# haliphinx/TCE-RVOS

Measured on AMD Instinct MI355X. Metric: clips/s (T=5, 360×640, Swin-T) at 1/2/4/8 MI355X; mask IoU vs ref, higher is better.
Workload: dtype f32 (3xf16-split MFMA, f32 accumulate); 1 GPU; swin_t_p4w7 T=5 360x640 + 32-token text, B=1 clip per forward, flags --with_box_refine --binary --f_token 8 --qtrans (BASELINE config 2); clips_in_flight_per_gpu=1, clips_per_forward=1, same_clip_in_group=False, ranks_per_gpu=1, parallelism=clip-sharded x1

## Files before the change

include/tce_rvos_debug.h:

```cpp
#ifndef TCE_RVOS_DEBUG_H
#define TCE_RVOS_DEBUG_H
#include <stdint.h>
#ifdef __cplusplus
extern "C" {
#endif
int tce_gemm_force_tile(int32_t tile);
int tce_debug_set_stamp_buffer(long long* dev_buf);
int tce_debug_set_epilogue(int32_t lds_staged);
int tce_debug_ffn_set_stamp_buffer(long long* dev_buf);
int tce_debug_ffn_set_half(int32_t mode);
int tce_debug_msda_set_lds(int32_t on);
int tce_debug_window_attn_set_mfma(int32_t on);
int tce_debug_mha_set_split(int32_t on);
int tce_debug_msda_set_fewq(int32_t on);
int tce_debug_conv3x3_set_waves(int32_t waves);
int tce_debug_conv3x3_set_pieces(int32_t pieces);
#ifdef __cplusplus
}
#endif
#endif
```

tce-rvos_amd/_lib.py:

```python
import ctypes as C
import os

HERE = os.path.dirname(os.path.abspath(__file__))
LIB_PATH = os.environ.get("TCE_LIB") or os.path.join(HERE, "lib", "libtce_rvos.so")

c_f = C.c_void_p
i32, i64, f32 = C.c_int32, C.c_int64, C.c_float


class GemmArgs(C.Structure):
    _fields_ = [("A", c_f), ("A2", c_f), ("W", c_f), ("bias", c_f), ("res", c_f), ("C", c_f),
                ("M", i32), ("N", i32), ("K", i32),
                ("lda", i32), ("lda2", i32), ("ldw", i32), ("ldc", i32), ("ldres", i32),
                ("act", i32), ("res_mode", i32), ("batch", i32),
                ("sA", i64), ("sA2", i64), ("sW", i64), ("sBias", i64), ("sC", i64), ("sRes", i64),
                ("conv", i32), ("T", i32), ("H", i32), ("Wd", i32), ("Cin", i32), ("Ho", i32), ("Wo", i32),
                ("kh", i32), ("kw", i32), ("stride", i32), ("pad", i32)]


class RowLinArgs(C.Structure):
    _fields_ = [("x", c_f), ("a2", c_f), ("packed", c_f), ("bias", c_f), ("res", c_f), ("out", c_f),
                ("g_in", c_f), ("be_in", c_f), ("g_out", c_f), ("be_out", c_f),
                ("ldx", i64), ("lda2", i64), ("ldres", i64), ("ldo", i64),
                ("sX", i64), ("sA2", i64), ("sRes", i64), ("sOut", i64),
# ... 92 lines not shown
    "tce_ffn_packed_bytes": (i64, [i32, i32]),
    "tce_ffn_pack_f32": (i32, [c_f, c_f, c_f, c_f, i32, i32, c_f]),
    "tce_ffn_fused_f32": (i32, [c_f, i64, c_f, c_f, c_f, c_f, f32, c_f, c_f, f32, c_f, i64, i32, i32, i32, i32, c_f]),
    "tce_ffn_split_ws_floats": (i64, [i32, i32, i32, i32]),
    "tce_ffn_split_counters": (i32, [i32, i32, i32, i32]),
    "tce_ffn_set_wg_cap": (i32, [i32]),
    "tce_ffn_capped_grid": (i32, [i32, i32, i32, C.POINTER(i32)]),
    "tce_ffn_fused_split_f32": (i32, [c_f, i64, c_f, c_f, c_f, c_f, f32, c_f, c_f, f32, c_f, i64, i32, i32, i32, i32, c_f, i64, c_f, i32, c_f]),
    "tce_xattn_prepare_f32": (i32, [c_f, c_f, c_f, c_f, c_f, c_f, c_f, i32, i32, i32, c_f]),
    "tce_ffn_pack_batched_f32": (i32, [c_f, c_f, c_f, c_f, i32, i32, i32, c_f]),
    "tce_xattn_fused_f32": (i32, [C.POINTER(XattnArgs), c_f]),
    "tce_xattn_ffn_fused_f32": (i32, [C.POINTER(XattnArgs), C.POINTER(XattnFfnArgs), c_f]),
    "tce_ffn_pack_chain_f32": (i32, [c_f, c_f, c_f, c_f, i32, i32, c_f]),
    "tce_xattn_pack_f32": (i32, [c_f, c_f, c_f, c_f, c_f, i32, i32, i32, c_f]),
    "tce_xattn_prepare_lens_f32": (i32, [c_f, c_f, c_f, c_f, c_f, c_f, c_f, i32, i32, i32, c_f, c_f]),
    "tce_xattn_pack_lens_f32": (i32, [c_f, c_f, c_f, c_f, c_f, i32, i32, i32, c_f, c_f]),
    "tce_rowlin_packed_bytes": (i64, [i32, i32]),
    "tce_rowlin_pack_f32": (i32, [c_f, i64, c_f, i32, i32, c_f]),
    "tce_rowlin_f32": (i32, [C.POINTER(RowLinArgs), c_f]),
    "tce_conv3x3_packed_bytes": (i64, [i32, i32]),
    "tce_conv3x3_pack_f32": (i32, [c_f, c_f, i32, i32, c_f]),
    "tce_conv3x3_f32": (i32, [c_f, i64, c_f, c_f, c_f, i64, i32, i32, i32, i32, i32, c_f]),
    "tce_conv3x3_split_ws_floats": (i64, [i32, i32, i32]),
    "tce_conv3x3_split_pieces": (i32, [i32, i32, i32]),
    "tce_conv3x3_split_kstep": (i32, [i32, i32]),
    "tce_conv3x3_split_f32": (i32, [c_f, i64, c_f, c_f, c_f, i64, i32, i32, i32, i32, i32, c_f, i64, c_f]),
    "tce_fewrow_linear_f32": (i32, [C.POINTER(FewRowArgs), c_f]),
    "tce_thin_linear_splits": (i32, [i32, i32, i32]),
    "tce_thin_partials_f32": (i32, [c_f, i64, i32, c_f, i32, c_f, i64, c_f, i32, i32, i32, c_f]),
    "tce_splitk_reduce_f32": (i32, [c_f, i32, i32, i32, c_f, i32, c_f, i32, i32, c_f, i32, c_f, c_f, f32, c_f]),
    "tce_mha_small64_splits_f32": (i32, [c_f, i32, c_f, c_f, i32, i32, f32, c_f]),
    "tce_swin_attn_packed_bytes": (i64, [i32]),
    "tce_swin_attn_pack_f32": (i32, [c_f, c_f, c_f, i32, c_f]),
    "tce_swin_attn_fused_f32": (i32, [c_f, i64, c_f, c_f, c_f, c_f, c_f, c_f, f32, c_f, i64, i32, i32, i32, i32, i32, c_f]),
    "tce_graph_begin": (i32, [c_f]),
    "tce_graph_end": (i32, [c_f, C.POINTER(C.c_void_p)]),
    "tce_graph_launch": (i32, [C.c_void_p, c_f]),
    "tce_graph_destroy": (i32, [C.c_void_p]),
    "tce_graph_group": (i32, [C.POINTER(C.c_void_p), i32, C.POINTER(C.c_void_p)]),
}

DEBUG_SIGNATURES = {
    "tce_gemm_force_tile": (i32, [i32]),
    "tce_debug_set_stamp_buffer": (i32, [c_f]),
    "tce_debug_set_epilogue": (i32, [i32]),
    "tce_debug_ffn_set_stamp_buffer": (i32, [c_f]),
    "tce_debug_ffn_set_half": (i32, [i32]),
    "tce_debug_msda_set_lds": (i32, [i32]),
    "tce_debug_window_attn_set_mfma": (i32, [i32]),
    "tce_debug_mha_set_split": (i32, [i32]),
    "tce_debug_msda_set_fewq": (i32, [i32]),
    "tce_debug_conv3x3_set_waves": (i32, [i32]),
    "tce_debug_conv3x3_set_pieces": (i32, [i32]),
}

VIDEO_SIGNATURES = {
    "tce_label_objects_u8": (i32, [C.POINTER(LabelObj), i32, c_f, c_f, i32, i32, i32, i32, i32, i32, i32, f32, f32, c_f]),
}

EVAL_SIGNATURES = {
    "tce_a2d_masks_u8": (i32, [c_f, c_f, i32, i32, i32, i32, i32, i32, i32, f32, c_f]),
    "tce_rle_ws_bytes": (i64, [i32, i32, i32]),
    "tce_rle_counts_u32": (i32, [c_f, c_f, c_f, c_f, i32, i32, i32, c_f]),
}

_LIB = None


class TceError(RuntimeError):
    pass


def lib():
    global _LIB
    if _LIB is None:
        if not os.path.exists(LIB_PATH):
            raise TceError(f"{LIB_PATH} not found: build the HIP extension first "
                           f"(python -c 'import __graft_entry__ as g; g.build()'); there is no fallback path")
        hwq = os.environ.get("GPU_MAX_HW_QUEUES")
        if hwq not in (None, "", "4"):
            import warnings
            warnings.warn(f"tce_rvos_amd: GPU_MAX_HW_QUEUES={hwq} is set; the HIP runtime's default (4) is the only value this "
                          f"launch program runs well with (1-3 crash the runtime, 5-16 double the clip time)", RuntimeWarning)
        l = C.CDLL(LIB_PATH)
        for name, (res, args) in list(SIGNATURES.items()) + list(DEBUG_SIGNATURES.items()) + list(VIDEO_SIGNATURES.items()) + \
                list(EVAL_SIGNATURES.items()):
            fn = getattr(l, name)
            fn.restype = res
            fn.argtypes = args
        _LIB = l
    return _LIB


def lib_raw():
    l = lib()
    return l.__dict__.get("_real", l)


def check(status, what=""):
    if status != 0:
        msg = lib().tce_last_error().decode(errors="replace")
        raise TceError(f"{what} failed ({status}): {msg}")
```

tce-rvos_amd/csrc/chain.hip:

```cpp
#include "common.h"
#include "gemm_epilogue.h"
#include "frag.h"
#include "../../include/tce_rvos.h"
#include "../../include/tce_rvos_debug.h"

namespace {

#ifndef FFN_ABL
#define FFN_ABL 0
#endif
static __device__ long long* g_ffn_stamps = nullptr;


template <int K, bool HAS_A2 = true>
__device__ __forceinline__ void load_x_frags(const float* __restrict__ x, const long long ldx,
                                             const float* __restrict__ a2, const long long lda2, const int a2_rows,
                                             const int m0, const int M, float* __restrict__ wt, const int lane,
                                             const float* __restrict__ g_in, const float* __restrict__ be_in,
                                             const float eps, h16x8 (&xh)[K / 16], h16x8 (&xl)[K / 16],
                                             const int single = 0) {
  constexpr int NP = K / 32;
  const int cr = lane >> 3, cp = (lane & 7) * 4;
  const int r = lane & 31, hf = lane >> 5;
  f32x4 v[NP][4];
// ... 1074 lines not shown
    } else {
      const int idx = (p_hi - 1 - 2 * KS) >> 1, t = idx >> 1, s2 = idx & 1, chunk = it - 1;
#pragma unroll
      for (int e = 0; e < 8; ++e) {
        const int col = 32 * chunk + 16 * s2 + 8 * (e >> 2) + 4 * hf + (e & 3);
        const int h = col / G, j = col - h * G;
        val[e] = (chunk >= 0 && chunk < NC && j < Lb) ? dot32(wo + (long long)(32 * t + r) * C + h * HD, v + j * C + h * HD) : 0.f;
      }
    }
    const HL f = split8(val, single);
    oh = __builtin_bit_cast(u32x4, f.hi);
    ol = __builtin_bit_cast(u32x4, f.lo);
  }
  stage_out[p_hi * 64 + lane] = oh;
  if (p_lo < P) stage_out[p_lo * 64 + lane] = ol;
}

constexpr int CONV_PAD_STAGES = 6;

struct ConvArgs {
  const float* x;
  const unsigned char* wpk;
  const float* bias;
  float* out;
  long long ldx, ldo;
  int H, W, M;
  int* range_flag;
  int single;
  int m_off;
  int nb, pieces;
  float* ws;
};

constexpr int CONV_ITERS = 12;
__host__ __device__ constexpr int conv3x3_piece_iter(const int pieces, const int s) { return s * CONV_ITERS / pieces; }

#ifndef CONV_ABL
#define CONV_ABL 0
#endif

template <int BYTE_OFF>
__device__ __forceinline__ void gload16(f32x4& dst, const float* ptr) {
  asm volatile("global_load_dwordx4 %0, %1, off offset:%2" : "=v"(dst) : "v"(ptr), "n"(BYTE_OFF) : "memory");
}

template <int I, int N, typename F>
__device__ __forceinline__ void static_for(F&& f) {
  if constexpr (I < N) {
    f(std::integral_constant<int, I>{});
    static_for<I + 1, N>(f);
  }
}

template <int CIN, bool SINGLE, int WAVES = 4, bool SPLIT = false>
__global__ void __launch_bounds__(64 * WAVES, WAVES / 4) conv3x3_kernel(const ConvArgs p) {
  constexpr int NTL = 8;
  constexpr int PW = 16 / WAVES;
  constexpr int STAGE = 2 * NTL * PIECE;
  constexpr int R = 4;
  constexpr int XS = WAVES == 4 ? 6 : 4, LX = XS + 1;
  constexpr int NW = WAVES == 4 ? CONV_PAD_STAGES - 2 : 3, LW = NW + 2;
  constexpr int INFLIGHT = (2 + PW) * (LW - 3);
  static_assert(LW <= CONV_PAD_STAGES, "the packed stream's zero padding covers the weight lead");
  constexpr int BODY = 12;
  constexpr int ITERS = 3 * (CIN / 64);
  constexpr int KS = BODY * ITERS;
  static_assert(CIN % 64 == 0, "channel chunks come in groups of four");
  static_assert(BODY % R == 0 && BODY % XS == 0 && BODY % NW == 0 && LX >= LW, "ring positions are compile-time");
  static_assert(WAVES * WT_BYTES <= R * STAGE, "the epilogue's staging tiles alias the ring");
  static_assert(!SPLIT || (ITERS == CONV_ITERS && WAVES == 4 && !SINGLE), "split pieces: CIN = 256, 128-pixel workgroups, split fp16");
  __shared__ __attribute__((aligned(16))) unsigned char smem[R * STAGE];

  const int tid = threadIdx.x, lane = tid & 63;
  const int wave = __builtin_amdgcn_readfirstlane(tid >> 6);
  const int hf = lane >> 5;
  const int blk = SPLIT ? (int)blockIdx.x % p.nb : (int)blockIdx.x;
  const int piece = SPLIT ? (int)blockIdx.x / p.nb : 0;
  const int i0 = SPLIT ? conv3x3_piece_iter(p.pieces, piece) : 0;
  const int i1 = SPLIT ? conv3x3_piece_iter(p.pieces, piece + 1) : ITERS;
  const int m0 = p.m_off + blk * (32 * WAVES) + wave * 32;

  const int m = m0 + (lane & 31);
  const int px = m % p.W, py = (m / p.W) % p.H;
  const float* const zeros = reinterpret_cast<const float*>(p.wpk + (long long)(KS + CONV_PAD_STAGES) * STAGE) + 8 * hf;
  const float* const xme = p.x + (long long)min(m, p.M - 1) * p.ldx + 8 * hf;
  auto iter_ptrs = [&](const int it, const float* (&q)[3]) {
    const int dy = it / (CIN / 64) - 1, cq = it % (CIN / 64);
    const bool row_ok = it < i1 && m < p.M && (unsigned)(py + dy) < (unsigned)p.H;
#pragma unroll
    for (int d = 0; d < 3; ++d) {
      const bool ok = row_ok && (unsigned)(px + d - 1) < (unsigned)p.W;
      q[d] = (ok ? xme + (long long)(dy * p.W + d - 1) * p.ldx : zeros) + 64 * cq;
    }
  };

  const float* wp = reinterpret_cast<const float*>(p.wpk + ((long long)i0 * BODY * STAGE) + (long long)(PW * wave) * PIECE + lane * 16);
  unsigned char* const wdst = smem + (PW * wave) * PIECE + lane * 16;
  f32x4 wr[NW][PW];
  auto wload = [&](f32x4 (&dst)[PW]) {
    if (!(CONV_ABL & 8)) {
      gload16<0>(dst[0], wp);
      gload16<PIECE>(dst[1], wp);
      if constexpr (PW == 4) {
        gload16<2 * PIECE>(dst[2], wp);
        gload16<3 * PIECE>(dst[3], wp);
      }
    }
    wp += STAGE / 4;
  };
  auto wstore = [&](const f32x4 (&src)[PW], const int stage) {
#pragma unroll
    for (int q = 0; q < PW; ++q) *reinterpret_cast<f32x4*>(wdst + stage * STAGE + q * PIECE) = src[q];
  };

  f32x4 xr[XS][2];
  const float* cur[3];
  const float* nxt[3];
  iter_ptrs(i0, cur);
  iter_ptrs(i0 + 1, nxt);
  auto xload = [&](auto jjc, f32x4 (&dst)[2]) {
    constexpr int JJ = decltype(jjc)::value;
    constexpr int J = JJ % BODY;
    const float* const src = JJ < BODY ? cur[J % 3] : nxt[J % 3];
    if (CONV_ABL & 16) return;
    gload16<64 * (J / 3)>(dst[0], src);
    gload16<64 * (J / 3) + 16>(dst[1], src);
  };
  auto wait_loads = [&](auto nc, f32x4 (&xs)[2], f32x4 (&ws)[PW]) {
    constexpr int N = (CONV_ABL & 24) ? 0 : decltype(nc)::value;
    if constexpr (PW == 4) {
      asm volatile("s_waitcnt vmcnt(%6)"
                   : "+v"(xs[0]), "+v"(xs[1]), "+v"(ws[0]), "+v"(ws[1]), "+v"(ws[2]), "+v"(ws[3])
                   : "n"(N)
                   : "memory");
    } else {
      asm volatile("s_waitcnt vmcnt(%4)" : "+v"(xs[0]), "+v"(xs[1]), "+v"(ws[0]), "+v"(ws[1]) : "n"(N) : "memory");
    }
  };
  using nfl = std::integral_constant<int, INFLIGHT>;

  f32x16 acc[NTL];
#pragma unroll
  for (int t = 0; t < NTL; ++t)
#pragma unroll
    for (int i = 0; i < 16; ++i) acc[t][i] = 0.f;
  h16x8 bh, bl;
  static_for<0, LX>([&](auto mc) {
    constexpr int m = decltype(mc)::value - LX;
    if constexpr (m + 2 >= 0) {
      wait_loads(nfl{}, xr[(m + 2) % XS], wr[(m + 2) % NW]);
      wstore(wr[(m + 2) % NW], (m + 2) % R);
      if constexpr (m + 2 == 0) {
        const float f[8] = {xr[0][0][0], xr[0][0][1], xr[0][0][2], xr[0][0][3], xr[0][1][0], xr[0][1][1], xr[0][1][2], xr[0][1][3]};
        const HL b = split8(f, SINGLE ? 1 : 0);
        bh = b.hi;
        bl = b.lo;
        asm volatile("" : "+v"(bh), "+v"(bl));
      }
    }
    if constexpr (m + LX >= 0) xload(std::integral_constant<int, m + LX>{}, xr[(m + LX) % XS]);
    if constexpr (m + LW >= 0) wload(wr[(m + LW) % NW]);
  });
  __syncthreads();
  h16x8 fh[4], fl[4];
  {
    const unsigned char* const st = smem + lane * 16;
    fh[0] = *reinterpret_cast<const h16x8*>(st);
    fl[0] = *reinterpret_cast<const h16x8*>(st + PIECE);
    fh[1] = *reinterpret_cast<const h16x8*>(st + 2 * PIECE);
    fl[1] = *reinterpret_cast<const h16x8*>(st + 3 * PIECE);
  }

  for (int it = i0; it < i1; ++it) {
    static_for<0, BODY>([&](auto jc) {
      constexpr int j = decltype(jc)::value;
      constexpr int nslot = (j + 1) % XS;
      const unsigned char* const st = smem + (j % R) * STAGE + lane * 16;
      unsigned nh[4], nl[4];
      auto tile = [&](auto tc) {
        constexpr int t = decltype(tc)::value;
#if CONV_ABL & 4
        const h16x8 k0 = fh[t % 4], k1 = fl[t % 4], k2 = bh, k3 = bl;
        asm volatile("" : : "v"(k0), "v"(k1), "v"(k2), "v"(k3));
#else
        if constexpr (!SINGLE) {
          acc[t] = __builtin_amdgcn_mfma_f32_32x32x16_f16(fh[t % 4], bl, acc[t], 0, 0, 0);
          acc[t] = __builtin_amdgcn_mfma_f32_32x32x16_f16(fl[t % 4], bh, acc[t], 0, 0, 0);
        }
        acc[t] = __builtin_amdgcn_mfma_f32_32x32x16_f16(fh[t % 4], bh, acc[t], 0, 0, 0);
#endif
      };
      static_for<0, 6>([&](auto tc) {
        constexpr int t = decltype(tc)::value;
        fh[(t + 2) % 4] = *reinterpret_cast<const h16x8*>(st + (2 * t + 4) * PIECE);
        fl[(t + 2) % 4] = *reinterpret_cast<const h16x8*>(st + (2 * t + 5) * PIECE);
        __builtin_amdgcn_sched_barrier(0);
        tile(tc);
        if constexpr (t < 4) {
          const float a = xr[nslot][t >> 1][2 * (t & 1)], b = xr[nslot][t >> 1][2 * (t & 1) + 1];
          if constexpr (SINGLE) {
            nh[t] = __builtin_bit_cast(unsigned, fp16x2_t{(__fp16)a, (__fp16)b});
            nl[t] = 0u;
          } else {
            const fp16x2_t h = __builtin_amdgcn_cvt_pkrtz(a, b);
            nh[t] = __builtin_bit_cast(unsigned, h);
            nl[t] = __builtin_bit_cast(unsigned, __builtin_amdgcn_cvt_pkrtz(a - (float)h[0], b - (float)h[1]));
          }
          asm volatile("" : "+v"(nh[t]), "+v"(nl[t]));
        }
        __builtin_amdgcn_sched_barrier(0);
      });
      wait_loads(nfl{}, xr[(j + 2) % XS], wr[(j + 2) % NW]);
      wstore(wr[(j + 2) % NW], (j + 2) % R);
      if (!(CONV_ABL & 2)) __syncthreads();
      xload(std::integral_constant<int, j + LX>{}, xr[(j + LX) % XS]);
      wload(wr[(j + LW) % NW]);
      {
        const unsigned char* const sn = smem + ((j + 1) % R) * STAGE + lane * 16;
        fh[0] = *reinterpret_cast<const h16x8*>(sn);
        fl[0] = *reinterpret_cast<const h16x8*>(sn + PIECE);
        fh[1] = *reinterpret_cast<const h16x8*>(sn + 2 * PIECE);
        fl[1] = *reinterpret_cast<const h16x8*>(sn + 3 * PIECE);
      }
      __builtin_amdgcn_sched_barrier(0);
      tile(std::integral_constant<int, 6>{});
      tile(std::integral_constant<int, 7>{});
      __builtin_amdgcn_sched_barrier(0);
      bh = __builtin_bit_cast(h16x8, u32x4{nh[0], nh[1], nh[2], nh[3]});
      bl = __builtin_bit_cast(h16x8, u32x4{nl[0], nl[1], nl[2], nl[3]});
    });
#pragma unroll
    for (int d = 0; d < 3; ++d) cur[d] = nxt[d];
    iter_ptrs(it + 2, nxt);
  }
  asm volatile("s_waitcnt vmcnt(0)" ::: "memory");
  __syncthreads();

  float* const wt = reinterpret_cast<float*>(smem + wave * WT_BYTES);
  tce_amax_t amax = 0;
  if constexpr (SPLIT) {
    float* const part = p.ws + (long long)piece * (p.M - p.m_off) * 256;
#pragma unroll
    for (int t = 0; t < NTL; ++t) tile_store(acc[t], part, 256, m0 - p.m_off, p.M - p.m_off, 32 * t, wt, lane, amax);
    return;
  }
  const ResTile none = {};
#pragma unroll
  for (int t = 0; t < NTL; ++t) {
    tile_bias_res<0>(acc[t], tile_bias_load(p.bias, 32 * t, lane), none, wt, lane);
    tile_store(acc[t], p.out, p.ldo, m0, p.M, 32 * t, wt, lane, amax);
  }
  tce_range_report(p.range_flag, amax);
}

__global__ void __launch_bounds__(256) conv3x3_reduce_kernel(const float* __restrict__ ws, const int pieces, const int rows,
                                                             const float* __restrict__ bias, float* __restrict__ out,
                                                             const long long ldo, const int m_off, int* range_flag) {
  const long long n4 = (long long)rows * 64, stride = (long long)gridDim.x * 256;
  tce_amax_t amax = 0;
  for (long long i = (long long)blockIdx.x * 256 + threadIdx.x; i < n4; i += stride) {
    const f32x4* src = reinterpret_cast<const f32x4*>(ws) + i;
    f32x4 v = src[0];
    for (int s = 1; s < pieces; ++s) v += src[(long long)s * n4];
    const int c4 = (int)(i & 63);
    if (bias) v += reinterpret_cast<const f32x4*>(bias)[c4];
    amax = tce_amax4(amax, v);
    *reinterpret_cast<f32x4*>(out + (m_off + (i >> 6)) * ldo + 4 * c4) = v;
  }
  tce_range_report(range_flag, amax);
}

__global__ void __launch_bounds__(256) conv3x3_pack_kernel(const float* __restrict__ w, unsigned char* __restrict__ out,
                                                           const int CIN, const long long units, const int single) {
  const long long u = (long long)blockIdx.x * 256 + threadIdx.x;
  if (u >= units) return;
  const int lane = (int)(u & 63);
  const long long pg = u >> 6;
  const int piece = (int)(pg & 15);
  const long long s = pg >> 4;
  const int r = lane & 31, hf = lane >> 5, t = piece >> 1;
  u32x4 o = {0u, 0u, 0u, 0u};
  if (s < 9 * CIN / 16) {
    const int it = (int)(s / 12), j = (int)(s % 12);
    const int dy = it / (CIN / 64), cc = 4 * (it % (CIN / 64)) + j / 3, dx = j % 3;
    float v[8];
#pragma unroll
// ... 433 lines not shown
                     (unsigned char*)packed, Cin, units, tce_gemm_single_pass());
  TCE_CHECK_LAUNCH("tce_conv3x3_pack_f32");
  return TCE_OK;
}

static int g_conv3_waves = 0;
extern "C" int tce_debug_conv3x3_set_waves(int32_t waves) {
  TCE_CHECK_ARG(waves == 0 || waves == 4 || waves == 8, "tce_debug_conv3x3_set_waves: 0 (automatic), 4 or 8");
  g_conv3_waves = waves;
  return TCE_OK;
}

struct Conv3Plan {
  int wide = 4;
  int full8 = 0;
  int m_narrow = 0;
  int nb = 0;
  int pieces = 1;
  long long ws_floats = 0;
};
inline Conv3Plan conv3x3_plan(const int M, const int cus, const int single, const int force_waves, const int split, const int force_pieces) {
  Conv3Plan pl;
  const int r4 = tce_cdiv(tce_cdiv(M, 128), cus), r8 = tce_cdiv(tce_cdiv(M, 256), cus);
  const int full8 = tce_cdiv(M, 256) / cus;
  const int rem_px = M - full8 * 256 * cus;
  const int mixed4 = 7 * full8 + 4 * tce_cdiv(tce_cdiv(rem_px, 128), cus);
  if (!force_waves && !single && full8 >= 1 && rem_px > 0 && mixed4 < 4 * r4 && mixed4 < 7 * r8) {
    pl.full8 = full8 * cus;
    pl.m_narrow = full8 * 256 * cus;
  } else {
    pl.wide = force_waves ? force_waves : (4 * r4 > 7 * r8 ? 8 : 4);
    if (single) pl.wide = 4;
    if (pl.wide == 8) return pl;
  }
  pl.nb = tce_cdiv(M - pl.m_narrow, 128);
  if (!split || single || pl.nb >= cus) return pl;
  const double OVH = 0.5, LAUNCH = 0.3, RED_BPI = 8.0 * (3u << 20);
  const long long px = M - pl.m_narrow;
  auto cost = [&](int p) {
    const double walk = (double)tce_cdiv((long long)pl.nb * p, cus) * (tce_cdiv(CONV_ITERS, p) + OVH);
    return p == 1 ? walk : walk + LAUNCH + (double)(p + 1) * px * 1024.0 / RED_BPI;
  };
  int best = 1;
  for (int p = 2; p <= 6; ++p)
    if ((long long)pl.nb * p <= 2ll * cus && cost(p) < cost(best)) best = p;
  if (force_pieces > 0) best = force_pieces;
  if (best > 1) {
    pl.pieces = best;
    pl.ws_floats = (long long)best * px * 256;
  }
  return pl;
}

static int g_conv3_pieces = 0;
extern "C" int tce_debug_conv3x3_set_pieces(int32_t pieces) {
  TCE_CHECK_ARG(pieces >= 0 && pieces <= CONV_ITERS, "tce_debug_conv3x3_set_pieces: 0 (automatic) .. 12");
  g_conv3_pieces = pieces;
  return TCE_OK;
}

static int conv3_force_waves() {
  static const int env_force = []() { const char* e = getenv("TCE_CONV3_WAVES"); return e ? atoi(e) : 0; }();
  return g_conv3_waves ? g_conv3_waves : env_force;
}

static Conv3Plan conv3x3_plan_for(const int M, const bool split) {
  return conv3x3_plan(M, tce_cu_count(), tce_gemm_single_pass(), conv3_force_waves(), split, g_conv3_pieces);
}

extern "C" int64_t tce_conv3x3_split_ws_floats(int32_t M, int32_t Cin, int32_t N) {
  return conv3x3_shape_ok(Cin, N) && M > 0 ? conv3x3_plan_for(M, true).ws_floats : 0;
}
extern "C" int32_t tce_conv3x3_split_pieces(int32_t M, int32_t Cin, int32_t N) {
  return conv3x3_shape_ok(Cin, N) && M > 0 ? conv3x3_plan_for(M, true).pieces : 0;
}
extern "C" int32_t tce_conv3x3_split_kstep(int32_t pieces, int32_t s) {
  return pieces >= 1 && pieces <= CONV_ITERS && s >= 0 && s <= pieces ? 12 * conv3x3_piece_iter(pieces, s) : -1;
}

static int conv3x3_launch(const float* x, int64_t ldx, const void* packed, const float* bias, float* out, int64_t ldo, int32_t T,
                          int32_t H, int32_t W, int32_t Cin, int32_t N, float* ws, int64_t ws_floats, const bool split, tceStream stream,
                          const char* name) {
  TCE_CHECK_ARG(conv3x3_shape_ok(Cin, N), "%s: unsupported shape Cin=%d N=%d (256 -> 256)", name, Cin, N);
  TCE_CHECK_ARG(x && packed && out && T > 0 && H > 0 && W > 0 && (long long)T * H * W < (1ll << 31),
                "%s: null pointer or bad sizes", name);
  TCE_CHECK_ARG(ldx >= Cin && ldx % 4 == 0 && ldo >= N && ldo % 4 == 0, "%s: bad row pitch", name);
  TCE_CHECK_ARG(tce_aligned16(x) && tce_aligned16(out) && tce_aligned16(packed) && (!bias || tce_aligned16(bias)),
                "%s: pointers must be 16-byte aligned", name);
  ConvArgs a;
  a.x = x; a.wpk = (const unsigned char*)packed; a.bias = bias; a.out = out;
  a.ldx = ldx; a.ldo = ldo; a.H = H; a.W = W; a.M = T * H * W;
  a.range_flag = tce_range_flag(); a.single = tce_gemm_single_pass();
  a.m_off = 0; a.nb = 0; a.pieces = 1; a.ws = nullptr;
  hipStream_t s = (hipStream_t)stream;
  const Conv3Plan pl = conv3x3_plan_for(a.M, split);
  if (pl.pieces > 1)
    TCE_CHECK_ARG(ws && tce_aligned16(ws) && ws_floats >= pl.ws_floats,
                  "%s: workspace of %lld floats needed (tce_conv3x3_split_ws_floats), %lld given", name, pl.ws_floats, (long long)ws_floats);
  if (pl.full8) hipLaunchKernelGGL((conv3x3_kernel<256, false, 8>), dim3(pl.full8), dim3(512), 0, s, a);
  a.m_off = pl.m_narrow;
  if (pl.wide == 8) hipLaunchKernelGGL((conv3x3_kernel<256, false, 8>), dim3(tce_cdiv(a.M, 256)), dim3(512), 0, s, a);
  else if (a.single) hipLaunchKernelGGL((conv3x3_kernel<256, true>), dim3(pl.nb), dim3(256), 0, s, a);
  else if (pl.pieces == 1) hipLaunchKernelGGL((conv3x3_kernel<256, false>), dim3(pl.nb), dim3(256), 0, s, a);
  else {
    a.nb = pl.nb; a.pieces = pl.pieces; a.ws = ws;
    hipLaunchKernelGGL((conv3x3_kernel<256, false, 4, true>), dim3(pl.nb * pl.pieces), dim3(256), 0, s, a);
    const int rows = a.M - a.m_off;
    hipLaunchKernelGGL(conv3x3_reduce_kernel, dim3(std::min(tce_cdiv((long long)rows * 64, 256), 8 * tce_cu_count())), dim3(256), 0, s,
                       (const float*)ws, pl.pieces, rows, bias, out, ldo, a.m_off, a.range_flag);
  }
  TCE_CHECK_LAUNCH(name);
  return TCE_OK;
}

extern "C" int tce_conv3x3_f32(const float* x, int64_t ldx, const void* packed, const float* bias, float* out, int64_t ldo,
                               int32_t T, int32_t H, int32_t W, int32_t Cin, int32_t N, tceStream stream) {
  return conv3x3_launch(x, ldx, packed, bias, out, ldo, T, H, W, Cin, N, nullptr, 0, false, stream, "tce_conv3x3_f32");
}

extern "C" int tce_conv3x3_split_f32(const float* x, int64_t ldx, const void* packed, const float* bias, float* out, int64_t ldo,
                                     int32_t T, int32_t H, int32_t W, int32_t Cin, int32_t N, float* ws, int64_t ws_floats,
                                     tceStream stream) {
  return conv3x3_launch(x, ldx, packed, bias, out, ldo, T, H, W, Cin, N, ws, ws_floats, true, stream, "tce_conv3x3_split_f32");
}

bool tce_patch_embed_mfma(const float* frames, const float* w, const float* b, const float* gamma, const float* beta,
                          float* out, int H, int W, int C, float eps, long long ntok, int Hp, int Wp, hipStream_t s) {
  if ((C != 96 && C != 128 && C != 192) || ntok >= (1ll << 31) || !tce_aligned16(frames) || !tce_aligned16(out) ||
      !tce_aligned16(w) || !tce_aligned16(b) || !tce_aligned16(gamma) || !tce_aligned16(beta))
    return false;
  const dim3 grid(tce_cdiv(ntok, 128)), block(256);
  int* const rf = tce_range_flag();
  const int single = tce_gemm_single_pass();
  if (C == 96) hipLaunchKernelGGL((patch_embed_mfma_kernel<3>), grid, block, 0, s, frames, w, b, gamma, beta, out, H, W, eps, (int)ntok, Hp, Wp, rf, single);
  else if (C == 128) hipLaunchKernelGGL((patch_embed_mfma_kernel<4>), grid, block, 0, s, frames, w, b, gamma, beta, out, H, W, eps, (int)ntok, Hp, Wp, rf, single);
  else hipLaunchKernelGGL((patch_embed_mfma_kernel<6>), grid, block, 0, s, frames, w, b, gamma, beta, out, H, W, eps, (int)ntok, Hp, Wp, rf, single);
  return true;
}
#endif
```

tce-rvos_amd/ops.py:

```python
import ctypes as C

import os
import threading

import torch

from ._lib import GemmArgs, check, lib

ACT_NONE, ACT_RELU, ACT_GELU, ACT_RELU_AFTER_RES = 0, 1, 2, 3
RES_NONE, RES_ADD, RES_MUL = 0, 1, 2


class Arena:

    ALIGN = 256
    FLAGS = 1 << 14

    def __init__(self, device, nbytes):
        self.device = torch.device(device)
        self.buf = torch.empty(int(nbytes), dtype=torch.uint8, device=self.device)
        self.off = 0
        self.peak = 0
        self.flags = torch.zeros(self.FLAGS, dtype=torch.int32, device=self.device)
        self.flag_off = 0
# ... 1043 lines not shown
    if nbytes < 0:
        raise ValueError(f"rowlin_pack: unsupported shape N={N} K={K}")
    out = torch.empty(nbytes, dtype=torch.uint8, device=w.device)
    check(lib().tce_rowlin_pack_f32(w.data_ptr(), ldw, out.data_ptr(), N, K, _stream()), "tce_rowlin_pack_f32")
    return out


def rowlin_register(w, table=None):
    if w.dim() != 2 or w.stride(1) != 1 or w.shape[1] not in ROWLIN_K or w.shape[0] % 32 or not w.is_cuda:
        return None
    r = _ROUTES if table is None else table
    key = (w.data_ptr(), w.shape[0], w.shape[1], w.stride(0), get_gemm_mode())
    if key not in r.rowlin:
        r.rowlin[key] = rowlin_pack(w)
        r.keep.append(w)
    return r.rowlin[key]


def rowlin(x, pk, out, M, N, K, ldx, ldo, bias=None, a2=None, lda2=0, a2_rows=0, act=ACT_NONE, res=None, ldres=0,
           res_mode=RES_NONE, ln_in=None, ln_out=None, eps_in=1e-5, eps_out=1e-5, batch=1, sX=0, sA2=0, sRes=0, sOut=0):
    from ._lib import RowLinArgs
    q = RowLinArgs()
    q.x, q.packed, q.out = x.data_ptr(), pk.data_ptr(), out.data_ptr()
    q.M, q.N, q.K, q.batch = M, N, K, batch
    q.ldx, q.ldo = ldx, ldo
    if a2 is not None:
        q.a2, q.lda2, q.a2_rows = a2.data_ptr(), lda2, a2_rows
    if bias is not None:
        q.bias = bias.data_ptr()
    if res_mode != RES_NONE:
        q.res, q.ldres = res.data_ptr(), ldres
    if ln_in is not None:
        q.g_in, q.be_in = ln_in[0].data_ptr(), ln_in[1].data_ptr()
    if ln_out is not None:
        q.g_out, q.be_out = ln_out[0].data_ptr(), ln_out[1].data_ptr()
    q.act, q.res_mode, q.eps_in, q.eps_out = act, res_mode, eps_in, eps_out
    q.sX, q.sA2, q.sRes, q.sOut = sX, sA2, sRes, sOut

    def go():
        check(lib().tce_rowlin_f32(C.byref(q), _stream()), "tce_rowlin_f32")
    if GEMM_PROFILE is None:
        go()
        return out
    e0, e1 = torch.cuda.Event(enable_timing=True), torch.cuda.Event(enable_timing=True)
    e0.record()
    go()
    e1.record()
    GEMM_PROFILE.append((f"rowlin_kernel<{K}", False, 2.0 * M * N * K * batch, e0, e1))
    return out


CONV3_MIN_PIXELS = int(os.environ.get("TCE_CONV3_MIN_PIXELS", 12000))
CONV3_SPLIT = os.environ.get("TCE_CONV3_SPLIT", "1") != "0"


def conv3x3_split_ws_floats(M, Cin=256, N=256):
    return int(lib().tce_conv3x3_split_ws_floats(M, Cin, N)) if CONV3_SPLIT else 0


def conv3x3_pack(w_cl, Cin):
    _chk(w_cl, "w")
    N = w_cl.shape[0]
    nbytes = lib().tce_conv3x3_packed_bytes(Cin, N)
    if nbytes < 0 or w_cl.shape[1] != 9 * Cin or not w_cl.is_contiguous():
        raise ValueError(f"conv3x3_pack: unsupported shape N={N} Cin={Cin}")
    out = torch.empty(nbytes, dtype=torch.uint8, device=w_cl.device)
    check(lib().tce_conv3x3_pack_f32(w_cl.data_ptr(), out.data_ptr(), Cin, N, _stream()), "tce_conv3x3_pack_f32")
    return out


def conv3x3_register(w_cl, Cin, table=None):
    if lib().tce_conv3x3_packed_bytes(Cin, w_cl.shape[0]) < 0 or w_cl.shape[1] != 9 * Cin:
        return None
    r = _ROUTES if table is None else table
    key = (w_cl.data_ptr(), w_cl.shape[0], w_cl.shape[1], get_gemm_mode())
    if key not in r.conv3:
        r.conv3[key] = conv3x3_pack(w_cl, Cin)
        r.keep.append(w_cl)
    return r.conv3[key]


def conv3x3(x, pk, T, H, W, Cin, N, bias=None, out=None, alloc=None):
    _chk(x, "x")
    M = T * H * W
    if out is None:
        out = alloc(M, N) if alloc else torch.empty(M, N, dtype=torch.float32, device=x.device)

    nws = conv3x3_split_ws_floats(M, Cin, N) if alloc else 0
    ws = alloc(nws) if nws else None

    def go():
        bp = bias.data_ptr() if bias is not None else None
        if ws is not None:
            check(lib().tce_conv3x3_split_f32(x.data_ptr(), x.stride(0), pk.data_ptr(), bp, out.data_ptr(), out.stride(0), T, H, W,
                                              Cin, N, ws.data_ptr(), nws, _stream()), "tce_conv3x3_split_f32")
        else:
            check(lib().tce_conv3x3_f32(x.data_ptr(), x.stride(0), pk.data_ptr(), bp, out.data_ptr(), out.stride(0), T, H, W, Cin,
                                        N, _stream()), "tce_conv3x3_f32")
    if GEMM_PROFILE is None:
        go()
        return out
    e0, e1 = torch.cuda.Event(enable_timing=True), torch.cuda.Event(enable_timing=True)
    e0.record()
    go()
    e1.record()
    GEMM_PROFILE.append((f"conv3x3_kernel<{Cin}", True, 2.0 * M * N * 9 * Cin, e0, e1))
    return out


XATTN_MIN_ROWS = int(os.environ.get("TCE_XATTN_MIN_ROWS", 4000))
XATTN_PACK_FUSED = os.environ.get("TCE_XATTN_PACK_FUSED", "1") != "0"


def xattn_static(wq, bq, scale=32 ** -0.5):
    return (torch.cat([wq.t(), bq[None]], 0) * scale).contiguous()


def xattn_pack(k, v, wqT_ext, wo, L, alloc, group=32, batch=1, lens=None):
    _chk(k, "k")
    _chk(v, "v")
    Hd = 8 * group
    if XATTN_PACK_FUSED:
        pk = alloc(batch, lib().tce_ffn_packed_bytes(256, Hd), dtype=torch.uint8)
        if lens is not None:
            check(lib().tce_xattn_pack_lens_f32(k.data_ptr(), v.data_ptr(), wqT_ext.data_ptr(), wo.data_ptr(), pk.data_ptr(), L, group,
                                                batch, lens.data_ptr(), _stream()), "tce_xattn_pack_lens_f32")
            return pk
        check(lib().tce_xattn_pack_f32(k.data_ptr(), v.data_ptr(), wqT_ext.data_ptr(), wo.data_ptr(), pk.data_ptr(), L, group, batch,
                                       _stream()), "tce_xattn_pack_f32")
        return pk
    W1, b1, W2 = alloc(batch, Hd, 256), alloc(batch, Hd), alloc(batch, 256, Hd)
    if lens is not None:
        check(lib().tce_xattn_prepare_lens_f32(k.data_ptr(), v.data_ptr(), wqT_ext.data_ptr(), wo.data_ptr(), W1.data_ptr(),
                                               b1.data_ptr(), W2.data_ptr(), L, group, batch, lens.data_ptr(), _stream()),
              "tce_xattn_prepare_lens_f32")
    else:
# ... 91 lines not shown
```

Measured before the change: 177.9 clips/s.

## Reuse centre-tap activations across 3x3 conv horizontal taps via DPP lane shifts

The 3x3 conv kernel now loads only the centre column of activations plus a single halo pixel at each end of the 32-pixel wave row, instead of three separate global loads per dy/channel chunk. The left and right taps come from DPP row shifts of the already split fp16 hi/lo values, with explicit zeroing at image borders. This cuts global activation traffic and VMEM requests roughly threefold. The cost is a new load/wait schedule built from constexpr in-flight counts, more registers, and extra DPP/select work. A runtime flag and env var can switch back to the old path.

```diff
diff --git a/include/tce_rvos_debug.h b/include/tce_rvos_debug.h
--- a/include/tce_rvos_debug.h
+++ b/include/tce_rvos_debug.h
@@ -15,6 +15,7 @@
 int tce_debug_msda_set_fewq(int32_t on);
 int tce_debug_conv3x3_set_waves(int32_t waves);
 int tce_debug_conv3x3_set_pieces(int32_t pieces);
+int tce_debug_conv3x3_set_reuse(int32_t reuse);
 #ifdef __cplusplus
 }
 #endif
diff --git a/tce-rvos_amd/_lib.py b/tce-rvos_amd/_lib.py
--- a/tce-rvos_amd/_lib.py
+++ b/tce-rvos_amd/_lib.py
@@ -168,6 +168,7 @@
     "tce_debug_msda_set_fewq": (i32, [i32]),
     "tce_debug_conv3x3_set_waves": (i32, [i32]),
     "tce_debug_conv3x3_set_pieces": (i32, [i32]),
+    "tce_debug_conv3x3_set_reuse": (i32, [i32]),
 }
 
 VIDEO_SIGNATURES = {
diff --git a/tce-rvos_amd/csrc/chain.hip b/tce-rvos_amd/csrc/chain.hip
--- a/tce-rvos_amd/csrc/chain.hip
+++ b/tce-rvos_amd/csrc/chain.hip
@@ -1150,7 +1150,26 @@
   }
 }
 
-template <int CIN, bool SINGLE, int WAVES = 4, bool SPLIT = false>
+template <int LW, int PW, bool PAIR>
+struct ConvReuse {
+  static constexpr int NC = PAIR ? 3 : 2;
+  static constexpr int centre(int c) { return 3 * (PAIR ? (c & ~1) : c) - LW - 1; }
+  static constexpr int halo(int c) { return 3 * c - LW; }
+  static constexpr int cslot(int c) { return PAIR ? ((c & 1) ? 1 + ((c >> 1) & 1) : 0) : (c & 1); }
+  static constexpr int loads(int k) {
+    int n = PW;
+    for (int c = -8; c < 16; ++c) n += 2 * (centre(c) == k) + 2 * (halo(c) == k);
+    return n;
+  }
+  static constexpr int inflight(int j) {
+    int n = 0;
+    for (int k = j + 3 - LW; k <= j - 1; ++k) n += loads(k);
+    return n;
+  }
+  static_assert(centre(-1) < -(LW + 1) && halo(-1) < -(LW + 1), "no request of an earlier iteration falls into the prologue");
+};
+
+template <int CIN, bool SINGLE, int WAVES = 4, bool SPLIT = false, bool REUSE = true>
 __global__ void __launch_bounds__(64 * WAVES, WAVES / 4) conv3x3_kernel(const ConvArgs p) {
   constexpr int NTL = 8;
   constexpr int PW = 16 / WAVES;
@@ -1159,6 +1178,7 @@
   constexpr int XS = WAVES == 4 ? 6 : 4, LX = XS + 1;
   constexpr int NW = WAVES == 4 ? CONV_PAD_STAGES - 2 : 3, LW = NW + 2;
   constexpr int INFLIGHT = (2 + PW) * (LW - 3);
+  using RU = ConvReuse<LW, PW, WAVES == 4>;
   static_assert(LW <= CONV_PAD_STAGES, "the packed stream's zero padding covers the weight lead");
   constexpr int BODY = 12;
   constexpr int ITERS = 3 * (CIN / 64);
@@ -1190,6 +1210,15 @@
       const bool ok = row_ok && (unsigned)(px + d - 1) < (unsigned)p.W;
       q[d] = (ok ? xme + (long long)(dy * p.W + d - 1) * p.ldx : zeros) + 64 * cq;
     }
+  };
+
+  const bool halo_l = (lane & 31) == 0, halo_r = (lane & 31) == 31, zero_l = px == 0 && !halo_l, zero_r = px == p.W - 1 && !halo_r;
+  auto reuse_ptrs = [&](const int it, const float*& qc, const float*& qh) {
+    const int dy = it / (CIN / 64) - 1, cq = it % (CIN / 64);
+    const bool row_ok = it < i1 && m < p.M && (unsigned)(py + dy) < (unsigned)p.H;
+    const bool hl = (lane & 31) == 0 && px > 0, hr = (lane & 31) == 31 && px < p.W - 1;
+    qc = (row_ok ? xme + (long long)(dy * p.W) * p.ldx : zeros) + 64 * cq;
+    qh = (row_ok && (hl || hr) ? xme + (long long)(dy * p.W + (hl ? -1 : 1)) * p.ldx : zeros) + 64 * cq;
   };
 
   const float* wp = reinterpret_cast<const float*>(p.wpk + ((long long)i0 * BODY * STAGE) + (long long)(PW * wave) * PIECE + lane * 16);
@@ -1214,8 +1243,10 @@
   f32x4 xr[XS][2];
   const float* cur[3];
   const float* nxt[3];
-  iter_ptrs(i0, cur);
-  iter_ptrs(i0 + 1, nxt);
+  if constexpr (!REUSE) {
+    iter_ptrs(i0, cur);
+    iter_ptrs(i0 + 1, nxt);
+  }
   auto xload = [&](auto jjc, f32x4 (&dst)[2]) {
     constexpr int JJ = decltype(jjc)::value;
     constexpr int J = JJ % BODY;
@@ -1223,6 +1254,81 @@
     if (CONV_ABL & 16) return;
     gload16<64 * (J / 3)>(dst[0], src);
     gload16<64 * (J / 3) + 16>(dst[1], src);
+  };
+  f32x4 craw[RU::NC][2], hraw[2][2];
+  unsigned cs_h[2][4], cs_l[2][4], rt_h[2][4], rt_l[2][4], lt_h[4], lt_l[4];
+  const float* ccur;
+  const float* cnxt;
+  const float* hcur;
+  const float* hnxt;
+  if constexpr (REUSE) {
+    reuse_ptrs(i0, ccur, hcur);
+    reuse_ptrs(i0 + 1, cnxt, hnxt);
+  }
+  auto reuse_loads = [&](auto kc) {
+    constexpr int K = decltype(kc)::value;
+    if (CONV_ABL & 16) return;
+    static_for<0, 8>([&](auto cc) {
+      constexpr int c = decltype(cc)::value;
+      if constexpr (RU::centre(c) == K && (K >= 0 || c < 4)) {
+        const float* const src = c < 4 ? ccur : cnxt;
+        gload16<64 * (c % 4)>(craw[RU::cslot(c)][0], src);
+        gload16<64 * (c % 4) + 16>(craw[RU::cslot(c)][1], src);
+      }
+    });
+    static_for<0, 8>([&](auto cc) {
+      constexpr int c = decltype(cc)::value;
+      if constexpr (RU::halo(c) == K && (K >= 0 || c < 4)) {
+        const float* const src = c < 4 ? hcur : hnxt;
+        gload16<64 * (c % 4)>(hraw[c & 1][0], src);
+        gload16<64 * (c % 4) + 16>(hraw[c & 1][1], src);
+      }
+    });
+  };
+  auto split2 = [&](const float a, const float b, unsigned& h, unsigned& l) {
+    if constexpr (SINGLE) {
+      h = __builtin_bit_cast(unsigned, fp16x2_t{(__fp16)a, (__fp16)b});
+      l = 0u;
+    } else {
+      const fp16x2_t hh = __builtin_amdgcn_cvt_pkrtz(a, b);
+      h = __builtin_bit_cast(unsigned, hh);
+      l = __builtin_bit_cast(unsigned, __builtin_amdgcn_cvt_pkrtz(a - (float)hh[0], b - (float)hh[1]));
+    }
+  };
+  auto reuse_centre = [&](auto cc, auto tc) {
+    constexpr int c = decltype(cc)::value, t = decltype(tc)::value;
+    f32x4(&raw)[2] = craw[RU::cslot(c)];
+    if constexpr (t == 0) asm volatile("" : "+v"(raw[0]), "+v"(raw[1]));
+    split2(raw[t >> 1][2 * (t & 1)], raw[t >> 1][2 * (t & 1) + 1], cs_h[c & 1][t], cs_l[c & 1][t]);
+    if constexpr (SINGLE) asm volatile("" : "+v"(cs_h[c & 1][t]));
+    else asm volatile("" : "+v"(cs_h[c & 1][t]), "+v"(cs_l[c & 1][t]));
+  };
+  auto reuse_taps = [&](auto cc, auto tc) {
+    constexpr int c = decltype(cc)::value, t = decltype(tc)::value;
+    f32x4(&raw)[2] = hraw[c & 1];
+    if constexpr (t == 0) asm volatile("" : "+v"(raw[0]), "+v"(raw[1]));
+    unsigned hh, hl;
+    split2(raw[t >> 1][2 * (t & 1)], raw[t >> 1][2 * (t & 1) + 1], hh, hl);
+    const int sh = (int)cs_h[c & 1][t], sl = (int)cs_l[c & 1][t];
+    const unsigned shr_h = (unsigned)__builtin_amdgcn_update_dpp(0, sh, 0x138 , 0xf, 0xf, false);
+    const unsigned shl_h = (unsigned)__builtin_amdgcn_update_dpp(0, sh, 0x130 , 0xf, 0xf, false);
+    lt_h[t] = halo_l ? hh : zero_l ? 0u : shr_h;
+    rt_h[c & 1][t] = halo_r ? hh : zero_r ? 0u : shl_h;
+    if constexpr (SINGLE) {
+      lt_l[t] = rt_l[c & 1][t] = 0u;
+      asm volatile("" : "+v"(lt_h[t]), "+v"(rt_h[c & 1][t]));
+    } else {
+      const unsigned shr_l = (unsigned)__builtin_amdgcn_update_dpp(0, sl, 0x138, 0xf, 0xf, false);
+      const unsigned shl_l = (unsigned)__builtin_amdgcn_update_dpp(0, sl, 0x130, 0xf, 0xf, false);
+      lt_l[t] = halo_l ? hl : zero_l ? 0u : shr_l;
+      rt_l[c & 1][t] = halo_r ? hl : zero_r ? 0u : shl_l;
+      asm volatile("" : "+v"(lt_h[t]), "+v"(lt_l[t]), "+v"(rt_h[c & 1][t]), "+v"(rt_l[c & 1][t]));
+    }
+  };
+  auto wait_weights = [&](auto nc, f32x4 (&ws)[PW]) {
+    constexpr int N = (CONV_ABL & 24) ? 0 : decltype(nc)::value;
+    if constexpr (PW == 4) asm volatile("s_waitcnt vmcnt(%4)" : "+v"(ws[0]), "+v"(ws[1]), "+v"(ws[2]), "+v"(ws[3]) : "n"(N) : "memory");
+    else asm volatile("s_waitcnt vmcnt(%2)" : "+v"(ws[0]), "+v"(ws[1]) : "n"(N) : "memory");
   };
   auto wait_loads = [&](auto nc, f32x4 (&xs)[2], f32x4 (&ws)[PW]) {
     constexpr int N = (CONV_ABL & 24) ? 0 : decltype(nc)::value;
@@ -1243,6 +1349,23 @@
 #pragma unroll
     for (int i = 0; i < 16; ++i) acc[t][i] = 0.f;
   h16x8 bh, bl;
+  if constexpr (REUSE) {
+    static_for<0, LW + 1>([&](auto mc) {
+      constexpr int m = decltype(mc)::value - (LW + 1);
+      if constexpr (m + 2 >= 0) {
+        wait_weights(std::integral_constant<int, RU::inflight(m)>{}, wr[(m + 2) % NW]);
+        wstore(wr[(m + 2) % NW], (m + 2) % R);
+        if constexpr (m + 2 == 0) {
+          static_for<0, 4>([&](auto tc) { reuse_centre(std::integral_constant<int, 0>{}, tc); });
+          static_for<0, 4>([&](auto tc) { reuse_taps(std::integral_constant<int, 0>{}, tc); });
+          bh = __builtin_bit_cast(h16x8, u32x4{lt_h[0], lt_h[1], lt_h[2], lt_h[3]});
+          bl = __builtin_bit_cast(h16x8, u32x4{lt_l[0], lt_l[1], lt_l[2], lt_l[3]});
+        }
+      }
+      reuse_loads(std::integral_constant<int, m>{});
+      if constexpr (m + LW >= 0) wload(wr[(m + LW) % NW]);
+    });
+  } else
   static_for<0, LX>([&](auto mc) {
     constexpr int m = decltype(mc)::value - LX;
     if constexpr (m + 2 >= 0) {
@@ -1294,7 +1417,10 @@
         fl[(t + 2) % 4] = *reinterpret_cast<const h16x8*>(st + (2 * t + 5) * PIECE);
         __builtin_amdgcn_sched_barrier(0);
         tile(tc);
-        if constexpr (t < 4) {
+        if constexpr (REUSE && t < 4) {
+          if constexpr (j % 3 == 1) reuse_centre(std::integral_constant<int, j / 3 + 1>{}, tc);
+          if constexpr (j % 3 == 2) reuse_taps(std::integral_constant<int, j / 3 + 1>{}, tc);
+        } else if constexpr (t < 4) {
           const float a = xr[nslot][t >> 1][2 * (t & 1)], b = xr[nslot][t >> 1][2 * (t & 1) + 1];
           if constexpr (SINGLE) {
             nh[t] = __builtin_bit_cast(unsigned, fp16x2_t{(__fp16)a, (__fp16)b});
@@ -1308,10 +1434,12 @@
         }
         __builtin_amdgcn_sched_barrier(0);
       });
-      wait_loads(nfl{}, xr[(j + 2) % XS], wr[(j + 2) % NW]);
+      if constexpr (REUSE) wait_weights(std::integral_constant<int, RU::inflight(j)>{}, wr[(j + 2) % NW]);
+      else wait_loads(nfl{}, xr[(j + 2) % XS], wr[(j + 2) % NW]);
       wstore(wr[(j + 2) % NW], (j + 2) % R);
       if (!(CONV_ABL & 2)) __syncthreads();
-      xload(std::integral_constant<int, j + LX>{}, xr[(j + LX) % XS]);
+      if constexpr (REUSE) reuse_loads(jc);
+      else xload(std::integral_constant<int, j + LX>{}, xr[(j + LX) % XS]);
       wload(wr[(j + LW) % NW]);
       {
         const unsigned char* const sn = smem + ((j + 1) % R) * STAGE + lane * 16;
@@ -1324,12 +1452,26 @@
       tile(std::integral_constant<int, 6>{});
       tile(std::integral_constant<int, 7>{});
       __builtin_amdgcn_sched_barrier(0);
-      bh = __builtin_bit_cast(h16x8, u32x4{nh[0], nh[1], nh[2], nh[3]});
-      bl = __builtin_bit_cast(h16x8, u32x4{nl[0], nl[1], nl[2], nl[3]});
+      if constexpr (REUSE) {
+        constexpr int c1 = ((j + 1) / 3) & 1;
+        const unsigned(&oh)[4] = (j + 1) % 3 == 0 ? lt_h : (j + 1) % 3 == 1 ? cs_h[c1] : rt_h[c1];
+        const unsigned(&ol)[4] = (j + 1) % 3 == 0 ? lt_l : (j + 1) % 3 == 1 ? cs_l[c1] : rt_l[c1];
+        bh = __builtin_bit_cast(h16x8, u32x4{oh[0], oh[1], oh[2], oh[3]});
+        bl = __builtin_bit_cast(h16x8, u32x4{ol[0], ol[1], ol[2], ol[3]});
+      } else {
+        bh = __builtin_bit_cast(h16x8, u32x4{nh[0], nh[1], nh[2], nh[3]});
+        bl = __builtin_bit_cast(h16x8, u32x4{nl[0], nl[1], nl[2], nl[3]});
+      }
     });
-#pragma unroll
-    for (int d = 0; d < 3; ++d) cur[d] = nxt[d];
-    iter_ptrs(it + 2, nxt);
+    if constexpr (REUSE) {
+      ccur = cnxt;
+      hcur = hnxt;
+      reuse_ptrs(it + 2, cnxt, hnxt);
+    } else {
+#pragma unroll
+      for (int d = 0; d < 3; ++d) cur[d] = nxt[d];
+      iter_ptrs(it + 2, nxt);
+    }
   }
   asm volatile("s_waitcnt vmcnt(0)" ::: "memory");
   __syncthreads();
@@ -1869,6 +2011,13 @@
   return pl;
 }
 
+static int g_conv3_reuse = 1;
+extern "C" int tce_debug_conv3x3_set_reuse(int32_t reuse) {
+  TCE_CHECK_ARG(reuse == 0 || reuse == 1, "tce_debug_conv3x3_set_reuse: 0 or 1");
+  g_conv3_reuse = reuse;
+  return TCE_OK;
+}
+
 static int g_conv3_pieces = 0;
 extern "C" int tce_debug_conv3x3_set_pieces(int32_t pieces) {
   TCE_CHECK_ARG(pieces >= 0 && pieces <= CONV_ITERS, "tce_debug_conv3x3_set_pieces: 0 (automatic) .. 12");
@@ -1914,14 +2063,24 @@
   if (pl.pieces > 1)
     TCE_CHECK_ARG(ws && tce_aligned16(ws) && ws_floats >= pl.ws_floats,
                   "%s: workspace of %lld floats needed (tce_conv3x3_split_ws_floats), %lld given", name, pl.ws_floats, (long long)ws_floats);
-  if (pl.full8) hipLaunchKernelGGL((conv3x3_kernel<256, false, 8>), dim3(pl.full8), dim3(512), 0, s, a);
+  auto launch = [&](auto single_c, auto waves_c, auto split_c, const int blocks) {
+    constexpr bool SG = decltype(single_c)::value, SP = decltype(split_c)::value;
+    constexpr int WV = decltype(waves_c)::value;
+    if (g_conv3_reuse) hipLaunchKernelGGL((conv3x3_kernel<256, SG, WV, SP, true>), dim3(blocks), dim3(64 * WV), 0, s, a);
+    else hipLaunchKernelGGL((conv3x3_kernel<256, SG, WV, SP, false>), dim3(blocks), dim3(64 * WV), 0, s, a);
+  };
+  using std::false_type;
+  using std::true_type;
+  using w4 = std::integral_constant<int, 4>;
+  using w8 = std::integral_constant<int, 8>;
+  if (pl.full8) launch(false_type{}, w8{}, false_type{}, pl.full8);
   a.m_off = pl.m_narrow;
-  if (pl.wide == 8) hipLaunchKernelGGL((conv3x3_kernel<256, false, 8>), dim3(tce_cdiv(a.M, 256)), dim3(512), 0, s, a);
-  else if (a.single) hipLaunchKernelGGL((conv3x3_kernel<256, true>), dim3(pl.nb), dim3(256), 0, s, a);
-  else if (pl.pieces == 1) hipLaunchKernelGGL((conv3x3_kernel<256, false>), dim3(pl.nb), dim3(256), 0, s, a);
+  if (pl.wide == 8) launch(false_type{}, w8{}, false_type{}, tce_cdiv(a.M, 256));
+  else if (a.single) launch(true_type{}, w4{}, false_type{}, pl.nb);
+  else if (pl.pieces == 1) launch(false_type{}, w4{}, false_type{}, pl.nb);
   else {
     a.nb = pl.nb; a.pieces = pl.pieces; a.ws = ws;
-    hipLaunchKernelGGL((conv3x3_kernel<256, false, 4, true>), dim3(pl.nb * pl.pieces), dim3(256), 0, s, a);
+    launch(false_type{}, w4{}, true_type{}, pl.nb * pl.pieces);
     const int rows = a.M - a.m_off;
     hipLaunchKernelGGL(conv3x3_reduce_kernel, dim3(std::min(tce_cdiv((long long)rows * 64, 256), 8 * tce_cu_count())), dim3(256), 0, s,
                        (const float*)ws, pl.pieces, rows, bias, out, ldo, a.m_off, a.range_flag);
diff --git a/tce-rvos_amd/ops.py b/tce-rvos_amd/ops.py
--- a/tce-rvos_amd/ops.py
+++ b/tce-rvos_amd/ops.py
@@ -1119,6 +1119,16 @@
 
 CONV3_MIN_PIXELS = int(os.environ.get("TCE_CONV3_MIN_PIXELS", 12000))
 CONV3_SPLIT = os.environ.get("TCE_CONV3_SPLIT", "1") != "0"
+_CONV3_REUSE_OFF = os.environ.get("TCE_CONV3_REUSE", "1") == "0"
+_conv3_reuse_applied = False
+
+
+def _apply_conv3_reuse():
+    global _conv3_reuse_applied
+    if not _conv3_reuse_applied:
+        _conv3_reuse_applied = True
+        if _CONV3_REUSE_OFF:
+            lib().tce_debug_conv3x3_set_reuse(0)
 
 
 def conv3x3_split_ws_floats(M, Cin=256, N=256):
@@ -1149,6 +1159,7 @@
 
 def conv3x3(x, pk, T, H, W, Cin, N, bias=None, out=None, alloc=None):
     _chk(x, "x")
+    _apply_conv3_reuse()
     M = T * H * W
     if out is None:
         out = alloc(M, N) if alloc else torch.empty(M, N, dtype=torch.float32, device=x.device)
```

Result: no change. 178.1 clips/s (median of 2 runs) (+0.1%).
